# G-U-N/Phased-Consistency-Model

Measured on NVIDIA H100. Metric: distillation steps/sec (SD1.5 PCM-LoRA, bs=8/GPU), higher is better.
Workload: dtype bf16

## Files before the change

pcm_b200/csrc/attn_wg.cu:

```cuda
#include "common.cuh"
#include "wgmma.cuh"
#include "host_common.h"

namespace pcm {

namespace {

constexpr int kAwThreads = 384;
constexpr int kAwStages = 2;
constexpr int kTile = 64 * 128;

struct alignas(64) AttnWgParams {
  CUtensorMap q_map, k_map, v_map;
  bf16* out;
  float* lse;
  int H, Sq, Skv, D;
  long long ldo;
  float c;
};

template <int KB>
__global__ void __launch_bounds__(kAwThreads, 1) attn_fwd_wg_kernel(const __grid_constant__ AttnWgParams p) {
  extern __shared__ uint8_t smem_raw[];
  uint8_t* smem = reinterpret_cast<uint8_t*>((reinterpret_cast<uintptr_t>(smem_raw) + 1023) &
                                             ~static_cast<uintptr_t>(1023));
  uint8_t* sQ = smem;
  uint8_t* sK = sQ + 2 * KB * kTile;
  uint8_t* sV = sK + kAwStages * KB * kTile;
  __shared__ __align__(8) uint64_t q_bar;
  __shared__ __align__(8) uint64_t full_bar[kAwStages];
  __shared__ __align__(8) uint64_t empty_bar[kAwStages];

  const int wg = threadIdx.x >> 7;
  const int b = blockIdx.z, h = blockIdx.y, q0 = blockIdx.x * 128;
  const int nblk = (p.Skv + 63) / 64;
  constexpr uint32_t kv_bytes = 2 * KB * kTile;

  if (threadIdx.x == 0) {
    tma_prefetch_desc(&p.q_map);
    tma_prefetch_desc(&p.k_map);
    tma_prefetch_desc(&p.v_map);
    mbar_init(&q_bar, 1);
    for (int i = 0; i < kAwStages; ++i) {
      mbar_init(&full_bar[i], 1);
      mbar_init(&empty_bar[i], 2);
    }
    fence_barrier_init();
  }
  __syncthreads();
  griddep_sync();

  if (wg == 0) {
    if (threadIdx.x == 0) {
      mbar_arrive_expect_tx(&q_bar, 2 * KB * kTile);
      for (int w = 0; w < 2; ++w)
        for (int kb = 0; kb < KB; ++kb)
          tma_load_3d(sQ + (w * KB + kb) * kTile, &p.q_map, &q_bar, h * p.D + kb * 64, q0 + 64 * w, b);
      for (int j = 0; j < nblk; ++j) {
        const int st = j % kAwStages;
        mbar_wait(&empty_bar[st], ((j / kAwStages) & 1) ^ 1);
        mbar_arrive_expect_tx(&full_bar[st], kv_bytes);
        for (int kb = 0; kb < KB; ++kb) {
          tma_load_3d(sK + (st * KB + kb) * kTile, &p.k_map, &full_bar[st], h * p.D + kb * 64, j * 64, b);
          tma_load_3d(sV + (st * KB + kb) * kTile, &p.v_map, &full_bar[st], h * p.D + kb * 64, j * 64, b);
        }
      }
    }
    return;
  }

  const int cw = wg - 1, et = threadIdx.x & 127, warp = et >> 5, lane = et & 31;
  uint8_t* myQ = sQ + cw * KB * kTile;
  mbar_wait(&q_bar, 0);
  if (p.D < KB * 64) {
    const int c0 = p.D >> 3, nch = KB * 8;
    for (int i = et; i < 64 * nch; i += 128) {
      const int row = i / nch, ch = i - row * nch;
      if (ch < c0) continue;
      const uint32_t a = smem_u32(myQ + (ch >> 3) * kTile) + row * 128 + (((ch & 7) ^ (row & 7)) << 4);
      sts128(a, 0u, 0u, 0u, 0u);
    }
    fence_proxy_async();
  }
  asm volatile("bar.sync %0, 128;" ::"r"(1 + cw) : "memory");

  float o[KB][32];
#pragma unroll
  for (int kb = 0; kb < KB; ++kb)
#pragma unroll
    for (int i = 0; i < 32; ++i) o[kb][i] = 0.f;
  float m_run[2] = {-INFINITY, -INFINITY}, l_run[2] = {0.f, 0.f};
  const uint32_t q_addr = smem_u32(myQ);

  for (int j = 0; j < nblk; ++j) {
    const int st = j % kAwStages;
    mbar_wait(&full_bar[st], (j / kAwStages) & 1);
    const uint32_t k_addr = smem_u32(sK + st * KB * kTile);
    const uint32_t v_addr = smem_u32(sV + st * KB * kTile);
    float s[32];
    wgmma_fence();
#pragma unroll
    for (int kb = 0; kb < KB; ++kb)
#pragma unroll
      for (int k = 0; k < 4; ++k)
        Wgmma<64, 0, 0>::mma(s, wgmma_desc_sw128(q_addr + kb * kTile + k * 32, 16, 1024),
                             wgmma_desc_sw128(k_addr + kb * kTile + k * 32, 16, 1024), (kb | k) != 0 ? 1u : 0u);
    wgmma_commit();
    wgmma_wait<0>();
    wgmma_fence_acc(s);

    const int kbase = j * 64 + 2 * (lane & 3);
    float mx[2] = {-INFINITY, -INFINITY};
#pragma unroll
    for (int i = 0; i < 32; ++i) {
      const int key = kbase + 8 * (i >> 2) + (i & 1);
      const float v = key < p.Skv ? s[i] * p.c : -INFINITY;
      s[i] = v;
      mx[(i >> 1) & 1] = fmaxf(mx[(i >> 1) & 1], v);
    }
    float alpha[2];
#pragma unroll
    for (int r = 0; r < 2; ++r) {
      mx[r] = fmaxf(mx[r], __shfl_xor_sync(0xffffffffu, mx[r], 1));
      mx[r] = fmaxf(mx[r], __shfl_xor_sync(0xffffffffu, mx[r], 2));
      const float mn = fmaxf(m_run[r], mx[r]);
      alpha[r] = exp2f(m_run[r] - mn);
      m_run[r] = mn;
    }
    float rs[2] = {0.f, 0.f};
    uint32_t pa[4][4];
#pragma unroll
    for (int i = 0; i < 32; i += 2) {
      const int r = (i >> 1) & 1;
      const float p0 = exp2f(s[i] - m_run[r]), p1 = exp2f(s[i + 1] - m_run[r]);
      rs[r] += p0 + p1;
      pa[i >> 3][(i & 7) >> 1] = pack_bf16x2(p0, p1);
    }
#pragma unroll
    for (int r = 0; r < 2; ++r) l_run[r] = l_run[r] * alpha[r] + rs[r];
#pragma unroll
    for (int kb = 0; kb < KB; ++kb)
#pragma unroll
      for (int i = 0; i < 32; ++i) o[kb][i] *= alpha[(i >> 1) & 1];

    wgmma_fence();
#pragma unroll
    for (int kk = 0; kk < 4; ++kk)
#pragma unroll
      for (int kb = 0; kb < KB; ++kb)
        wgmma_rs_m64n64<1>(o[kb], pa[kk], wgmma_desc_sw128(v_addr + kb * kTile + kk * 2048, kTile, 1024), 1u);
    wgmma_commit();
    wgmma_wait<0>();
#pragma unroll
    for (int kb = 0; kb < KB; ++kb) wgmma_fence_acc(o[kb]);
    __syncwarp();
    if (et == 0) mbar_arrive(&empty_bar[st]);
  }

#pragma unroll
  for (int r = 0; r < 2; ++r) {
    l_run[r] += __shfl_xor_sync(0xffffffffu, l_run[r], 1);
    l_run[r] += __shfl_xor_sync(0xffffffffu, l_run[r], 2);
  }
  const int row0 = q0 + 64 * cw + 16 * warp + (lane >> 2);
#pragma unroll
  for (int r = 0; r < 2; ++r) {
    const int row = row0 + 8 * r;
    if (row >= p.Sq) continue;
    const float inv = 1.f / l_run[r];
    bf16* orow = p.out + (static_cast<long long>(b) * p.Sq + row) * p.ldo + h * p.D;
#pragma unroll
    for (int kb = 0; kb < KB; ++kb)
#pragma unroll
      for (int q = 0; q < 8; ++q) {
        const int col = kb * 64 + 8 * q + 2 * (lane & 3);
        if (col < p.D)
          *reinterpret_cast<uint32_t*>(orow + col) =
              pack_bf16x2(o[kb][4 * q + 2 * r] * inv, o[kb][4 * q + 2 * r + 1] * inv);
      }
    if ((lane & 3) == 0 && p.lse) p.lse[(static_cast<long long>(b) * p.H + h) * p.Sq + row] = m_run[r] + log2f(l_run[r]);
  }
}

struct alignas(64) AttnBwdParams {
  CUtensorMap fix0_map, fix1_map;
  CUtensorMap str0_map, str1_map;
  const float *lse, *delta;
  bf16 *out0, *out1;
  long long ld0, ld1;
  int H, Sq, Skv, D;
  int n_fix, n_str;
  float c, scale;
};

template <bool KV>
__global__ void __launch_bounds__(kAwThreads, 1) attn_bwd_wg_kernel(const __grid_constant__ AttnBwdParams p) {
  extern __shared__ uint8_t smem_raw[];
  uint8_t* smem = reinterpret_cast<uint8_t*>((reinterpret_cast<uintptr_t>(smem_raw) + 1023) &
                                             ~static_cast<uintptr_t>(1023));
  uint8_t* sF = smem;
  uint8_t* sS = sF + 4 * kTile;
  __shared__ __align__(8) uint64_t f_bar;
// ... 108 lines not shown
#pragma unroll
      for (int e = 0; e < 2; ++e) {
        const int col = 8 * (i >> 2) + 2 * (lane & 3) + e;
        float l, d;
        bool ok;
        if (KV) {
          l = lc[2 * (i >> 2) + e];
          d = dc[2 * (i >> 2) + e];
          ok = rvalid[r];
        } else {
          l = lrow[r];
          d = drow[r];
          ok = j * 64 + col < p.Skv;
        }
        pv[e] = ok ? exp2f(s[i + e] * p.c - l) : 0.f;
        g[e] = pv[e] * (dp[i + e] - d);
      }
      pa[i >> 3][(i & 7) >> 1] = pack_bf16x2(pv[0], pv[1]);
      dsa[i >> 3][(i & 7) >> 1] = pack_bf16x2(g[0], g[1]);
    }
    wgmma_fence();
#pragma unroll
    for (int kk = 0; kk < 4; ++kk) {
      wgmma_rs_m64n64<1>(acc0, dsa[kk], wgmma_desc_sw128(s0 + kk * 2048, kTile, 1024), 1u);
      if (KV) wgmma_rs_m64n64<1>(acc1, pa[kk], wgmma_desc_sw128(s1 + kk * 2048, kTile, 1024), 1u);
    }
    wgmma_commit();
    wgmma_wait<0>();
    wgmma_fence_acc(acc0);
    wgmma_fence_acc(acc1);
    __syncwarp();
    if (et == 0) mbar_arrive(&empty_bar[st]);
  }

#pragma unroll
  for (int r = 0; r < 2; ++r) {
    if (!rvalid[r]) continue;
    const long long row = static_cast<long long>(b) * p.n_fix + frow + 8 * r;
    bf16* o0 = p.out0 + row * p.ld0 + col0;
    bf16* o1 = KV ? p.out1 + row * p.ld1 + col0 : nullptr;
#pragma unroll
    for (int q = 0; q < 8; ++q) {
      const int col = 8 * q + 2 * (lane & 3);
      if (col < p.D) {
        *reinterpret_cast<uint32_t*>(o0 + col) =
            pack_bf16x2(acc0[4 * q + 2 * r] * p.scale, acc0[4 * q + 2 * r + 1] * p.scale);
        if (KV) *reinterpret_cast<uint32_t*>(o1 + col) = pack_bf16x2(acc1[4 * q + 2 * r], acc1[4 * q + 2 * r + 1]);
      }
    }
  }
}

int encode_seq_map(CUtensorMap* m, const void* base, int HD, int S, int B, long long ld) {
  if ((reinterpret_cast<uintptr_t>(base) & 15) != 0 || (ld & 7) != 0)
    return set_error("attention: tensor map base not 16-byte aligned or row stride not a multiple of 8");
  cuuint64_t dims[3] = {static_cast<cuuint64_t>(HD), static_cast<cuuint64_t>(S), static_cast<cuuint64_t>(B)};
  cuuint64_t strides[2] = {static_cast<cuuint64_t>(ld) * 2, static_cast<cuuint64_t>(ld) * 2 * S};
  cuuint32_t box[3] = {64, 64, 1}, estr[3] = {1, 1, 1};
  return encode_tmap(m, base, 3, dims, strides, box, estr);
}

}

int attn_fwd_wg(const void* q, const void* k, const void* v, void* out, float* lse, int B, int H, int Sq,
                int Skv, int D, long long ldq, long long ldk, long long ldv, long long ldo, float scale,
                cudaStream_t stream) {
  if (D % 8 != 0 || D > 128) return 1;
  static AttnWgParams p;
  memset(&p, 0, sizeof(p));
  int rc;
  if ((rc = encode_seq_map(&p.q_map, q, H * D, Sq, B, ldq)) != 0) return rc;
  if ((rc = encode_seq_map(&p.k_map, k, H * D, Skv, B, ldk)) != 0) return rc;
  if ((rc = encode_seq_map(&p.v_map, v, H * D, Skv, B, ldv)) != 0) return rc;
  p.out = reinterpret_cast<bf16*>(out);
  p.lse = lse;
  p.H = H; p.Sq = Sq; p.Skv = Skv; p.D = D; p.ldo = ldo;
  p.c = scale * 1.4426950408889634f;
  const dim3 grid((Sq + 127) / 128, H, B);
  if (D <= 64) {
    const size_t smem = (2 + 2 * kAwStages) * kTile + 1024;
    static bool attr = false;
    if (!attr) {
      CUDA_TRY(cudaFuncSetAttribute(attn_fwd_wg_kernel<1>, cudaFuncAttributeMaxDynamicSharedMemorySize,
                                    static_cast<int>(smem)));
      attr = true;
    }
    CUDA_TRY(launch_pdl(attn_fwd_wg_kernel<1>, grid, dim3(kAwThreads), smem, stream, p));
  } else {
    const size_t smem = 2 * (2 + 2 * kAwStages) * kTile + 1024;
    static bool attr = false;
    if (!attr) {
      CUDA_TRY(cudaFuncSetAttribute(attn_fwd_wg_kernel<2>, cudaFuncAttributeMaxDynamicSharedMemorySize,
                                    static_cast<int>(smem)));
      attr = true;
    }
    CUDA_TRY(launch_pdl(attn_fwd_wg_kernel<2>, grid, dim3(kAwThreads), smem, stream, p));
  }
  CUDA_TRY(cudaGetLastError());
  return 0;
}

int attn_bwd_wg(const void* q, const void* k, const void* v, const void* dout, const float* lse,
                const float* delta, void* dq, void* dk, void* dv, int B, int H, int Sq, int Skv, int D,
                long long ldq, long long ldk, long long ldv, long long ldo, float scale, cudaStream_t stream) {
  if (D % 8 != 0 || D > 64) return 1;
  static AttnBwdParams pk, pq;
  memset(&pk, 0, sizeof(pk));
  int rc;
  if ((rc = encode_seq_map(&pk.fix0_map, k, H * D, Skv, B, ldk)) != 0) return rc;
  if ((rc = encode_seq_map(&pk.fix1_map, v, H * D, Skv, B, ldv)) != 0) return rc;
  if ((rc = encode_seq_map(&pk.str0_map, q, H * D, Sq, B, ldq)) != 0) return rc;
  if ((rc = encode_seq_map(&pk.str1_map, dout, H * D, Sq, B, ldo)) != 0) return rc;
  pk.lse = lse; pk.delta = delta;
  pk.H = H; pk.Sq = Sq; pk.Skv = Skv; pk.D = D;
  pk.c = scale * 1.4426950408889634f;
  pq = pk;
  pk.out0 = reinterpret_cast<bf16*>(dk); pk.ld0 = ldk;
  pk.out1 = reinterpret_cast<bf16*>(dv); pk.ld1 = ldv;
  pk.n_fix = Skv; pk.n_str = Sq; pk.scale = scale;
  pq.fix0_map = pk.str0_map; pq.fix1_map = pk.str1_map;
// ... 21 lines not shown
```

pcm_b200/csrc/common.cuh:

```cuda
#pragma once
#include <cuda.h>
#include <cuda_bf16.h>
#include <cuda_runtime.h>
#include <stdint.h>

namespace pcm {

typedef __nv_bfloat16 bf16;

__device__ __forceinline__ uint32_t smem_u32(const void* p) {
  return static_cast<uint32_t>(__cvta_generic_to_shared(p));
}

__device__ __forceinline__ void sts128(uint32_t addr, uint32_t a, uint32_t b, uint32_t c, uint32_t d) {
  asm volatile("st.shared.v4.b32 [%0], {%1, %2, %3, %4};" ::"r"(addr), "r"(a), "r"(b), "r"(c), "r"(d)
               : "memory");
}
__device__ __forceinline__ float4 lds128(uint32_t addr) {
  float4 v;
  asm volatile("ld.shared.v4.f32 {%0, %1, %2, %3}, [%4];"
               : "=f"(v.x), "=f"(v.y), "=f"(v.z), "=f"(v.w)
               : "r"(addr)
               : "memory");
  return v;
// ... 119 lines not shown
__device__ __forceinline__ void wgmma_fence_acc(float (&d)[R]) {
#pragma unroll
  for (int i = 0; i < R; ++i) asm volatile("" : "+f"(d[i])::"memory");
}

template <int R>
__device__ __forceinline__ void regs_dealloc() {
  asm volatile("setmaxnreg.dec.sync.aligned.u32 %0;" ::"n"(R));
}
template <int R>
__device__ __forceinline__ void regs_alloc() {
  asm volatile("setmaxnreg.inc.sync.aligned.u32 %0;" ::"n"(R));
}

__device__ __forceinline__ uint64_t wgmma_desc_sw128(uint32_t smem_addr, uint32_t lbo_bytes,
                                                     uint32_t sbo_bytes) {
  uint64_t d = 0;
  d |= static_cast<uint64_t>((smem_addr & 0x3FFFF) >> 4);
  d |= static_cast<uint64_t>((lbo_bytes >> 4) & 0x3FFF) << 16;
  d |= static_cast<uint64_t>((sbo_bytes >> 4) & 0x3FFF) << 32;
  d |= static_cast<uint64_t>(1) << 62;
  return d;
}

__device__ __forceinline__ void red_add_v4(float* addr, float a, float b, float c, float d) {
  asm volatile("red.global.add.v4.f32 [%0], {%1, %2, %3, %4};" ::"l"(addr), "f"(a), "f"(b), "f"(c), "f"(d)
               : "memory");
}

__device__ __forceinline__ uint32_t pack_bf16x2(float a, float b) {
  __nv_bfloat162 h = __floats2bfloat162_rn(a, b);
  return *reinterpret_cast<uint32_t*>(&h);
}
__device__ __forceinline__ float2 unpack_bf16x2(uint32_t u) {
  __nv_bfloat162 h = *reinterpret_cast<__nv_bfloat162*>(&u);
  return __bfloat1622float2(h);
}
__device__ __forceinline__ float warp_sum(float v) {
#pragma unroll
  for (int o = 16; o > 0; o >>= 1) v += __shfl_xor_sync(0xffffffffu, v, o);
  return v;
}
__device__ __forceinline__ float warp_max(float v) {
#pragma unroll
  for (int o = 16; o > 0; o >>= 1) v = fmaxf(v, __shfl_xor_sync(0xffffffffu, v, o));
  return v;
}
__device__ __forceinline__ float frcp_approx(float d) {
  float r;
  asm("rcp.approx.ftz.f32 %0, %1;" : "=f"(r) : "f"(d));
  return r;
}
__device__ __forceinline__ float sigmoid_f(float x) { return frcp_approx(1.f + __expf(-x)); }
__device__ __forceinline__ float silu_f(float x) { return x * sigmoid_f(x); }
__device__ __forceinline__ float dsilu_f(float x) {
  const float s = sigmoid_f(x);
  return s * (1.f + x * (1.f - s));
}

}
```

pcm_b200/csrc/host_common.cu:

```cuda
#include "host_common.h"
#include <stdio.h>
#include <stdlib.h>
#include <cudaTypedefs.h>
#include "../../include/pcm_b200.h"

namespace pcm {

static thread_local char g_err[512] = "";

int set_error(const char* msg) {
  snprintf(g_err, sizeof(g_err), "%s", msg);
  return -1;
}
int set_cuda_error(cudaError_t e, const char* what) {
  snprintf(g_err, sizeof(g_err), "CUDA error %d (%s) at %s", static_cast<int>(e),
           cudaGetErrorString(e), what);
  return -2;
}
bool pdl_enabled() {
  static int v = -1;
  if (v < 0) v = getenv("PCM_NO_PDL") ? 0 : 1;
  return v == 1;
}
int num_sms() {
// ... 13 lines not shown
                             CUtensorMapL2promotion, CUtensorMapFloatOOBfill);

static EncodeFn get_encode() {
  static EncodeFn fn = nullptr;
  if (!fn) {
    void* p = nullptr;
    cudaDriverEntryPointQueryResult q;
    if (cudaGetDriverEntryPoint("cuTensorMapEncodeTiled", &p, cudaEnableDefault, &q) ==
            cudaSuccess &&
        q == cudaDriverEntryPointSuccess)
      fn = reinterpret_cast<EncodeFn>(p);
  }
  return fn;
}

int encode_tmap(CUtensorMap* map, const void* base, int rank, const cuuint64_t* dims,
                const cuuint64_t* strides_bytes, const cuuint32_t* box, const cuuint32_t* estr,
                int swizzle_bytes) {
  EncodeFn fn = get_encode();
  if (!fn) return set_error("cuTensorMapEncodeTiled entry point unavailable (no CUDA driver?)");
  CUresult r = fn(map, CU_TENSOR_MAP_DATA_TYPE_BFLOAT16, static_cast<cuuint32_t>(rank),
                  const_cast<void*>(base), dims, strides_bytes, box, estr,
                  CU_TENSOR_MAP_INTERLEAVE_NONE,
                  swizzle_bytes == 64 ? CU_TENSOR_MAP_SWIZZLE_64B : CU_TENSOR_MAP_SWIZZLE_128B,
                  CU_TENSOR_MAP_L2_PROMOTION_L2_256B, CU_TENSOR_MAP_FLOAT_OOB_FILL_NONE);
  if (r != CUDA_SUCCESS) {
    char buf[256];
    snprintf(buf, sizeof(buf),
             "cuTensorMapEncodeTiled failed (%d): rank %d dims [%llu,%llu,%llu,%llu] box "
             "[%u,%u,%u,%u] stride0 %llu",
             static_cast<int>(r), rank, (unsigned long long)dims[0],
             (unsigned long long)(rank > 1 ? dims[1] : 0), (unsigned long long)(rank > 2 ? dims[2] : 0),
             (unsigned long long)(rank > 3 ? dims[3] : 0), box[0], rank > 1 ? box[1] : 0,
             rank > 2 ? box[2] : 0, rank > 3 ? box[3] : 0, (unsigned long long)strides_bytes[0]);
    return set_error(buf);
  }
  return 0;
}

const char* last_error() { return g_err; }

}

extern "C" const char* pcm_last_error(void) { return pcm::last_error(); }
extern "C" int pcm_version(void) { return 1; }
extern "C" int pcm_num_sms(void) { return pcm::num_sms(); }
```

pcm_b200/csrc/wgmma.cuh:

```cuda
#pragma once
#include <stdint.h>

namespace pcm {

template <int N, int TA, int TB>
struct Wgmma;

template <int TA, int TB>
struct Wgmma<32, TA, TB> {
  __device__ __forceinline__ static void mma(float (&d)[16], uint64_t a, uint64_t b, uint32_t acc) {
    asm volatile(
        "{\n\t.reg .pred p;\n\t"
        "setp.ne.b32 p, %18, 0;\n\t"
        "wgmma.mma_async.sync.aligned.m64n32k16.f32.bf16.bf16 "
        "{%0, %1, %2, %3, %4, %5, %6, %7, %8, %9, %10, %11, %12, %13, %14, %15}, "
        "%16, %17, p, 1, 1, %19, %20;\n\t}"
        : "+f"(d[0]), "+f"(d[1]), "+f"(d[2]), "+f"(d[3]), "+f"(d[4]), "+f"(d[5]), "+f"(d[6]), "+f"(d[7]), "+f"(d[8]), "+f"(d[9]), "+f"(d[10]), "+f"(d[11]), "+f"(d[12]), "+f"(d[13]), "+f"(d[14]), "+f"(d[15])
        : "l"(a), "l"(b), "r"(acc), "n"(TA), "n"(TB));
  }
};

template <int TA, int TB>
struct Wgmma<64, TA, TB> {
  __device__ __forceinline__ static void mma(float (&d)[32], uint64_t a, uint64_t b, uint32_t acc) {
// ... 72 lines not shown
        "setp.ne.b32 p, %114, 0;\n\t"
        "wgmma.mma_async.sync.aligned.m64n224k16.f32.bf16.bf16 "
        "{%0, %1, %2, %3, %4, %5, %6, %7, %8, %9, %10, %11, %12, %13, %14, %15, %16, %17, %18, %19, %20, %21, %22, %23, %24, %25, %26, %27, %28, %29, %30, %31, %32, %33, %34, %35, %36, %37, %38, %39, %40, %41, %42, %43, %44, %45, %46, %47, %48, %49, %50, %51, %52, %53, %54, %55, %56, %57, %58, %59, %60, %61, %62, %63, %64, %65, %66, %67, %68, %69, %70, %71, %72, %73, %74, %75, %76, %77, %78, %79, %80, %81, %82, %83, %84, %85, %86, %87, %88, %89, %90, %91, %92, %93, %94, %95, %96, %97, %98, %99, %100, %101, %102, %103, %104, %105, %106, %107, %108, %109, %110, %111}, "
        "%112, %113, p, 1, 1, %115, %116;\n\t}"
        : "+f"(d[0]), "+f"(d[1]), "+f"(d[2]), "+f"(d[3]), "+f"(d[4]), "+f"(d[5]), "+f"(d[6]), "+f"(d[7]), "+f"(d[8]), "+f"(d[9]), "+f"(d[10]), "+f"(d[11]), "+f"(d[12]), "+f"(d[13]), "+f"(d[14]), "+f"(d[15]), "+f"(d[16]), "+f"(d[17]), "+f"(d[18]), "+f"(d[19]), "+f"(d[20]), "+f"(d[21]), "+f"(d[22]), "+f"(d[23]), "+f"(d[24]), "+f"(d[25]), "+f"(d[26]), "+f"(d[27]), "+f"(d[28]), "+f"(d[29]), "+f"(d[30]), "+f"(d[31]), "+f"(d[32]), "+f"(d[33]), "+f"(d[34]), "+f"(d[35]), "+f"(d[36]), "+f"(d[37]), "+f"(d[38]), "+f"(d[39]), "+f"(d[40]), "+f"(d[41]), "+f"(d[42]), "+f"(d[43]), "+f"(d[44]), "+f"(d[45]), "+f"(d[46]), "+f"(d[47]), "+f"(d[48]), "+f"(d[49]), "+f"(d[50]), "+f"(d[51]), "+f"(d[52]), "+f"(d[53]), "+f"(d[54]), "+f"(d[55]), "+f"(d[56]), "+f"(d[57]), "+f"(d[58]), "+f"(d[59]), "+f"(d[60]), "+f"(d[61]), "+f"(d[62]), "+f"(d[63]), "+f"(d[64]), "+f"(d[65]), "+f"(d[66]), "+f"(d[67]), "+f"(d[68]), "+f"(d[69]), "+f"(d[70]), "+f"(d[71]), "+f"(d[72]), "+f"(d[73]), "+f"(d[74]), "+f"(d[75]), "+f"(d[76]), "+f"(d[77]), "+f"(d[78]), "+f"(d[79]), "+f"(d[80]), "+f"(d[81]), "+f"(d[82]), "+f"(d[83]), "+f"(d[84]), "+f"(d[85]), "+f"(d[86]), "+f"(d[87]), "+f"(d[88]), "+f"(d[89]), "+f"(d[90]), "+f"(d[91]), "+f"(d[92]), "+f"(d[93]), "+f"(d[94]), "+f"(d[95]), "+f"(d[96]), "+f"(d[97]), "+f"(d[98]), "+f"(d[99]), "+f"(d[100]), "+f"(d[101]), "+f"(d[102]), "+f"(d[103]), "+f"(d[104]), "+f"(d[105]), "+f"(d[106]), "+f"(d[107]), "+f"(d[108]), "+f"(d[109]), "+f"(d[110]), "+f"(d[111])
        : "l"(a), "l"(b), "r"(acc), "n"(TA), "n"(TB));
  }
};

template <int TA, int TB>
struct Wgmma<256, TA, TB> {
  __device__ __forceinline__ static void mma(float (&d)[128], uint64_t a, uint64_t b, uint32_t acc) {
    asm volatile(
        "{\n\t.reg .pred p;\n\t"
        "setp.ne.b32 p, %130, 0;\n\t"
        "wgmma.mma_async.sync.aligned.m64n256k16.f32.bf16.bf16 "
        "{%0, %1, %2, %3, %4, %5, %6, %7, %8, %9, %10, %11, %12, %13, %14, %15, %16, %17, %18, %19, %20, %21, %22, %23, %24, %25, %26, %27, %28, %29, %30, %31, %32, %33, %34, %35, %36, %37, %38, %39, %40, %41, %42, %43, %44, %45, %46, %47, %48, %49, %50, %51, %52, %53, %54, %55, %56, %57, %58, %59, %60, %61, %62, %63, %64, %65, %66, %67, %68, %69, %70, %71, %72, %73, %74, %75, %76, %77, %78, %79, %80, %81, %82, %83, %84, %85, %86, %87, %88, %89, %90, %91, %92, %93, %94, %95, %96, %97, %98, %99, %100, %101, %102, %103, %104, %105, %106, %107, %108, %109, %110, %111, %112, %113, %114, %115, %116, %117, %118, %119, %120, %121, %122, %123, %124, %125, %126, %127}, "
        "%128, %129, p, 1, 1, %131, %132;\n\t}"
        : "+f"(d[0]), "+f"(d[1]), "+f"(d[2]), "+f"(d[3]), "+f"(d[4]), "+f"(d[5]), "+f"(d[6]), "+f"(d[7]), "+f"(d[8]), "+f"(d[9]), "+f"(d[10]), "+f"(d[11]), "+f"(d[12]), "+f"(d[13]), "+f"(d[14]), "+f"(d[15]), "+f"(d[16]), "+f"(d[17]), "+f"(d[18]), "+f"(d[19]), "+f"(d[20]), "+f"(d[21]), "+f"(d[22]), "+f"(d[23]), "+f"(d[24]), "+f"(d[25]), "+f"(d[26]), "+f"(d[27]), "+f"(d[28]), "+f"(d[29]), "+f"(d[30]), "+f"(d[31]), "+f"(d[32]), "+f"(d[33]), "+f"(d[34]), "+f"(d[35]), "+f"(d[36]), "+f"(d[37]), "+f"(d[38]), "+f"(d[39]), "+f"(d[40]), "+f"(d[41]), "+f"(d[42]), "+f"(d[43]), "+f"(d[44]), "+f"(d[45]), "+f"(d[46]), "+f"(d[47]), "+f"(d[48]), "+f"(d[49]), "+f"(d[50]), "+f"(d[51]), "+f"(d[52]), "+f"(d[53]), "+f"(d[54]), "+f"(d[55]), "+f"(d[56]), "+f"(d[57]), "+f"(d[58]), "+f"(d[59]), "+f"(d[60]), "+f"(d[61]), "+f"(d[62]), "+f"(d[63]), "+f"(d[64]), "+f"(d[65]), "+f"(d[66]), "+f"(d[67]), "+f"(d[68]), "+f"(d[69]), "+f"(d[70]), "+f"(d[71]), "+f"(d[72]), "+f"(d[73]), "+f"(d[74]), "+f"(d[75]), "+f"(d[76]), "+f"(d[77]), "+f"(d[78]), "+f"(d[79]), "+f"(d[80]), "+f"(d[81]), "+f"(d[82]), "+f"(d[83]), "+f"(d[84]), "+f"(d[85]), "+f"(d[86]), "+f"(d[87]), "+f"(d[88]), "+f"(d[89]), "+f"(d[90]), "+f"(d[91]), "+f"(d[92]), "+f"(d[93]), "+f"(d[94]), "+f"(d[95]), "+f"(d[96]), "+f"(d[97]), "+f"(d[98]), "+f"(d[99]), "+f"(d[100]), "+f"(d[101]), "+f"(d[102]), "+f"(d[103]), "+f"(d[104]), "+f"(d[105]), "+f"(d[106]), "+f"(d[107]), "+f"(d[108]), "+f"(d[109]), "+f"(d[110]), "+f"(d[111]), "+f"(d[112]), "+f"(d[113]), "+f"(d[114]), "+f"(d[115]), "+f"(d[116]), "+f"(d[117]), "+f"(d[118]), "+f"(d[119]), "+f"(d[120]), "+f"(d[121]), "+f"(d[122]), "+f"(d[123]), "+f"(d[124]), "+f"(d[125]), "+f"(d[126]), "+f"(d[127])
        : "l"(a), "l"(b), "r"(acc), "n"(TA), "n"(TB));
  }
};

template <int TB>
__device__ __forceinline__ void wgmma_rs_m64n64(float (&d)[32], const uint32_t (&a)[4], uint64_t b, uint32_t acc) {
  asm volatile(
      "{\n\t.reg .pred p;\n\t"
      "setp.ne.b32 p, %37, 0;\n\t"
      "wgmma.mma_async.sync.aligned.m64n64k16.f32.bf16.bf16 "
      "{%0, %1, %2, %3, %4, %5, %6, %7, %8, %9, %10, %11, %12, %13, %14, %15, %16, %17, %18, %19, %20, %21, %22, %23, %24, %25, %26, %27, %28, %29, %30, %31}, "
      "{%32, %33, %34, %35}, %36, p, 1, 1, %38;\n\t}"
      : "+f"(d[0]), "+f"(d[1]), "+f"(d[2]), "+f"(d[3]), "+f"(d[4]), "+f"(d[5]), "+f"(d[6]), "+f"(d[7]), "+f"(d[8]), "+f"(d[9]), "+f"(d[10]), "+f"(d[11]), "+f"(d[12]), "+f"(d[13]), "+f"(d[14]), "+f"(d[15]), "+f"(d[16]), "+f"(d[17]), "+f"(d[18]), "+f"(d[19]), "+f"(d[20]), "+f"(d[21]), "+f"(d[22]), "+f"(d[23]), "+f"(d[24]), "+f"(d[25]), "+f"(d[26]), "+f"(d[27]), "+f"(d[28]), "+f"(d[29]), "+f"(d[30]), "+f"(d[31])
      : "r"(a[0]), "r"(a[1]), "r"(a[2]), "r"(a[3]), "l"(b), "r"(acc), "n"(TB));
}

}
```

Before: 6.343.

## Pipeline QK and PV wgmma in attention forward with head-dim-specialized tiles

Restructures the wgmma attention forward kernel so that the QK^T matmul of block j overlaps the PV matmul of block j-1, and deepens the TMA K/V pipeline to four stages. The kernel is now templated on the padded head dim, using a single wide RS wgmma over V loaded with 32B-swizzled 16-column boxes, and three consumer warpgroups when the head dim is at most 64. It also adds warp-specialized register reallocation, ex2.approx.ftz exponentials, masking only on a ragged final block, and skipping the output rescale when the running max is unchanged. The cost is more shared memory, heavier register pressure, and more complex barrier accounting.

After: 6.617, median of 6. 4.3% higher.

```diff
diff --git a/pcm_b200/csrc/attn_wg.cu b/pcm_b200/csrc/attn_wg.cu
--- a/pcm_b200/csrc/attn_wg.cu
+++ b/pcm_b200/csrc/attn_wg.cu
@@ -8,7 +8,9 @@
 
 constexpr int kAwThreads = 384;
 constexpr int kAwStages = 2;
+constexpr int kFwdStages = 4;
 constexpr int kTile = 64 * 128;
+constexpr int kVBox = 64 * 32;
 
 struct alignas(64) AttnWgParams {
   CUtensorMap q_map, k_map, v_map;
@@ -19,31 +21,43 @@
   float c;
 };
 
-template <int KB>
-__global__ void __launch_bounds__(kAwThreads, 1) attn_fwd_wg_kernel(const __grid_constant__ AttnWgParams p) {
+__host__ __device__ constexpr int fwd_consumers(int DP) { return DP <= 64 ? 3 : 2; }
+
+template <int DP>
+constexpr size_t attn_fwd_smem() {
+  return fwd_consumers(DP) * ((DP + 63) / 64) * kTile + kFwdStages * (((DP + 63) / 64) * kTile + (DP / 16) * kVBox) +
+         1024;
+}
+
+template <int DP>
+__global__ void __launch_bounds__(128 * (fwd_consumers(DP) + 1), 1)
+    attn_fwd_wg_kernel(const __grid_constant__ AttnWgParams p) {
+  constexpr int NC = fwd_consumers(DP);
+  constexpr int KB = (DP + 63) / 64;
+  constexpr int NV = DP / 16;
+  constexpr int kKBytes = KB * kTile, kVBytes = NV * kVBox;
   extern __shared__ uint8_t smem_raw[];
   uint8_t* smem = reinterpret_cast<uint8_t*>((reinterpret_cast<uintptr_t>(smem_raw) + 1023) &
                                              ~static_cast<uintptr_t>(1023));
   uint8_t* sQ = smem;
-  uint8_t* sK = sQ + 2 * KB * kTile;
-  uint8_t* sV = sK + kAwStages * KB * kTile;
+  uint8_t* sK = sQ + NC * kKBytes;
+  uint8_t* sV = sK + kFwdStages * kKBytes;
   __shared__ __align__(8) uint64_t q_bar;
-  __shared__ __align__(8) uint64_t full_bar[kAwStages];
-  __shared__ __align__(8) uint64_t empty_bar[kAwStages];
+  __shared__ __align__(8) uint64_t full_bar[kFwdStages];
+  __shared__ __align__(8) uint64_t empty_bar[kFwdStages];
 
   const int wg = threadIdx.x >> 7;
-  const int b = blockIdx.z, h = blockIdx.y, q0 = blockIdx.x * 128;
+  const int b = blockIdx.z, h = blockIdx.y, q0 = blockIdx.x * 64 * NC;
   const int nblk = (p.Skv + 63) / 64;
-  constexpr uint32_t kv_bytes = 2 * KB * kTile;
 
   if (threadIdx.x == 0) {
     tma_prefetch_desc(&p.q_map);
     tma_prefetch_desc(&p.k_map);
     tma_prefetch_desc(&p.v_map);
     mbar_init(&q_bar, 1);
-    for (int i = 0; i < kAwStages; ++i) {
+    for (int i = 0; i < kFwdStages; ++i) {
       mbar_init(&full_bar[i], 1);
-      mbar_init(&empty_bar[i], 2);
+      mbar_init(&empty_bar[i], NC);
     }
     fence_barrier_init();
   }
@@ -51,26 +65,28 @@
   griddep_sync();
 
   if (wg == 0) {
+    regs_dealloc<NC == 3 ? 32 : 40>();
     if (threadIdx.x == 0) {
-      mbar_arrive_expect_tx(&q_bar, 2 * KB * kTile);
-      for (int w = 0; w < 2; ++w)
+      mbar_arrive_expect_tx(&q_bar, NC * kKBytes);
+      for (int w = 0; w < NC; ++w)
         for (int kb = 0; kb < KB; ++kb)
           tma_load_3d(sQ + (w * KB + kb) * kTile, &p.q_map, &q_bar, h * p.D + kb * 64, q0 + 64 * w, b);
       for (int j = 0; j < nblk; ++j) {
-        const int st = j % kAwStages;
-        mbar_wait(&empty_bar[st], ((j / kAwStages) & 1) ^ 1);
-        mbar_arrive_expect_tx(&full_bar[st], kv_bytes);
-        for (int kb = 0; kb < KB; ++kb) {
-          tma_load_3d(sK + (st * KB + kb) * kTile, &p.k_map, &full_bar[st], h * p.D + kb * 64, j * 64, b);
-          tma_load_3d(sV + (st * KB + kb) * kTile, &p.v_map, &full_bar[st], h * p.D + kb * 64, j * 64, b);
-        }
+        const int st = j % kFwdStages;
+        mbar_wait(&empty_bar[st], ((j / kFwdStages) & 1) ^ 1);
+        mbar_arrive_expect_tx(&full_bar[st], kKBytes + kVBytes);
+        for (int kb = 0; kb < KB; ++kb)
+          tma_load_3d(sK + st * kKBytes + kb * kTile, &p.k_map, &full_bar[st], h * p.D + kb * 64, j * 64, b);
+        for (int n = 0; n < NV; ++n)
+          tma_load_3d(sV + st * kVBytes + n * kVBox, &p.v_map, &full_bar[st], h * p.D + n * 16, j * 64, b);
       }
     }
     return;
   }
 
+  regs_alloc<NC == 3 ? 160 : 232>();
   const int cw = wg - 1, et = threadIdx.x & 127, warp = et >> 5, lane = et & 31;
-  uint8_t* myQ = sQ + cw * KB * kTile;
+  uint8_t* myQ = sQ + cw * kKBytes;
   mbar_wait(&q_bar, 0);
   if (p.D < KB * 64) {
     const int c0 = p.D >> 3, nch = KB * 8;
@@ -84,78 +100,102 @@
   }
   asm volatile("bar.sync %0, 128;" ::"r"(1 + cw) : "memory");
 
-  float o[KB][32];
-#pragma unroll
-  for (int kb = 0; kb < KB; ++kb)
-#pragma unroll
-    for (int i = 0; i < 32; ++i) o[kb][i] = 0.f;
+  float o[DP / 2];
+#pragma unroll
+  for (int i = 0; i < DP / 2; ++i) o[i] = 0.f;
   float m_run[2] = {-INFINITY, -INFINITY}, l_run[2] = {0.f, 0.f};
   const uint32_t q_addr = smem_u32(myQ);
-
-  for (int j = 0; j < nblk; ++j) {
-    const int st = j % kAwStages;
-    mbar_wait(&full_bar[st], (j / kAwStages) & 1);
-    const uint32_t k_addr = smem_u32(sK + st * KB * kTile);
-    const uint32_t v_addr = smem_u32(sV + st * KB * kTile);
-    float s[32];
+  const float c = p.c;
+  const bool ragged = (p.Skv & 63) != 0;
+
+  auto issue_qk = [&](float (&s)[32], int st) {
+    const uint32_t k_addr = smem_u32(sK + st * kKBytes);
     wgmma_fence();
 #pragma unroll
-    for (int kb = 0; kb < KB; ++kb)
-#pragma unroll
-      for (int k = 0; k < 4; ++k)
-        Wgmma<64, 0, 0>::mma(s, wgmma_desc_sw128(q_addr + kb * kTile + k * 32, 16, 1024),
-                             wgmma_desc_sw128(k_addr + kb * kTile + k * 32, 16, 1024), (kb | k) != 0 ? 1u : 0u);
+    for (int k = 0; k < DP / 16; ++k)
+      Wgmma<64, 0, 0>::mma(s, wgmma_desc_sw128(q_addr + (k >> 2) * kTile + (k & 3) * 32, 16, 1024),
+                           wgmma_desc_sw128(k_addr + (k >> 2) * kTile + (k & 3) * 32, 16, 1024), k != 0 ? 1u : 0u);
     wgmma_commit();
-    wgmma_wait<0>();
-    wgmma_fence_acc(s);
-
-    const int kbase = j * 64 + 2 * (lane & 3);
+  };
+  auto issue_pv = [&](const uint32_t (&pa)[4][4], int st) {
+    const uint32_t v_addr = smem_u32(sV + st * kVBytes);
+    wgmma_fence();
+#pragma unroll
+    for (int kk = 0; kk < 4; ++kk) WgmmaRS<DP, 1>::mma(o, pa[kk], wgmma_desc_sw32(v_addr + kk * 512, kVBox, 256), 1u);
+    wgmma_commit();
+  };
+  auto softmax = [&](float (&s)[32], int j, float (&alpha)[2], float (&rs)[2]) {
+#pragma unroll
+    for (int i = 0; i < 32; ++i) s[i] *= c;
+    if (ragged && j == nblk - 1) {
+      const int kbase = j * 64 + 2 * (lane & 3);
+#pragma unroll
+      for (int i = 0; i < 32; ++i)
+        if (kbase + 8 * (i >> 2) + (i & 1) >= p.Skv) s[i] = -INFINITY;
+    }
     float mx[2] = {-INFINITY, -INFINITY};
 #pragma unroll
-    for (int i = 0; i < 32; ++i) {
-      const int key = kbase + 8 * (i >> 2) + (i & 1);
-      const float v = key < p.Skv ? s[i] * p.c : -INFINITY;
-      s[i] = v;
-      mx[(i >> 1) & 1] = fmaxf(mx[(i >> 1) & 1], v);
-    }
-    float alpha[2];
+    for (int i = 0; i < 32; ++i) mx[(i >> 1) & 1] = fmaxf(mx[(i >> 1) & 1], s[i]);
+    float nm[2];
 #pragma unroll
     for (int r = 0; r < 2; ++r) {
       mx[r] = fmaxf(mx[r], __shfl_xor_sync(0xffffffffu, mx[r], 1));
       mx[r] = fmaxf(mx[r], __shfl_xor_sync(0xffffffffu, mx[r], 2));
       const float mn = fmaxf(m_run[r], mx[r]);
-      alpha[r] = exp2f(m_run[r] - mn);
+      alpha[r] = ex2_ftz(m_run[r] - mn);
       m_run[r] = mn;
-    }
-    float rs[2] = {0.f, 0.f};
-    uint32_t pa[4][4];
+      nm[r] = -mn;
+      rs[r] = 0.f;
+    }
 #pragma unroll
     for (int i = 0; i < 32; i += 2) {
       const int r = (i >> 1) & 1;
-      const float p0 = exp2f(s[i] - m_run[r]), p1 = exp2f(s[i + 1] - m_run[r]);
-      rs[r] += p0 + p1;
-      pa[i >> 3][(i & 7) >> 1] = pack_bf16x2(p0, p1);
-    }
+      s[i] = ex2_ftz(s[i] + nm[r]);
+      s[i + 1] = ex2_ftz(s[i + 1] + nm[r]);
+      rs[r] += s[i] + s[i + 1];
+    }
+  };
+  auto pack = [&](uint32_t (&pa)[4][4], const float (&s)[32]) {
+#pragma unroll
+    for (int i = 0; i < 32; i += 2) pa[i >> 3][(i & 7) >> 1] = pack_bf16x2(s[i], s[i + 1]);
+  };
+
+  uint32_t pa[4][4];
+  {
+    mbar_wait(&full_bar[0], 0);
+    float s[32], alpha[2], rs[2];
+    issue_qk(s, 0);
+    wgmma_wait<0>();
+    wgmma_fence_acc(s);
+    softmax(s, 0, alpha, rs);
+    pack(pa, s);
+#pragma unroll
+    for (int r = 0; r < 2; ++r) l_run[r] = rs[r];
+  }
+  for (int j = 1; j < nblk; ++j) {
+    const int st = j % kFwdStages, pst = (j - 1) % kFwdStages;
+    mbar_wait(&full_bar[st], (j / kFwdStages) & 1);
+    float s[32], alpha[2], rs[2];
+    issue_qk(s, st);
+    issue_pv(pa, pst);
+    wgmma_wait<1>();
+    wgmma_fence_acc(s);
+    softmax(s, j, alpha, rs);
+    wgmma_wait<0>();
+    wgmma_fence_acc(o);
+    __syncwarp();
+    if (et == 0) mbar_arrive(&empty_bar[pst]);
 #pragma unroll
     for (int r = 0; r < 2; ++r) l_run[r] = l_run[r] * alpha[r] + rs[r];
-#pragma unroll
-    for (int kb = 0; kb < KB; ++kb)
-#pragma unroll
-      for (int i = 0; i < 32; ++i) o[kb][i] *= alpha[(i >> 1) & 1];
-
-    wgmma_fence();
-#pragma unroll
-    for (int kk = 0; kk < 4; ++kk)
-#pragma unroll
-      for (int kb = 0; kb < KB; ++kb)
-        wgmma_rs_m64n64<1>(o[kb], pa[kk], wgmma_desc_sw128(v_addr + kb * kTile + kk * 2048, kTile, 1024), 1u);
-    wgmma_commit();
-    wgmma_wait<0>();
-#pragma unroll
-    for (int kb = 0; kb < KB; ++kb) wgmma_fence_acc(o[kb]);
-    __syncwarp();
-    if (et == 0) mbar_arrive(&empty_bar[st]);
-  }
+    if (!__all_sync(0xffffffffu, alpha[0] == 1.f && alpha[1] == 1.f)) {
+#pragma unroll
+      for (int i = 0; i < DP / 2; ++i) o[i] *= alpha[(i >> 1) & 1];
+    }
+    pack(pa, s);
+  }
+  issue_pv(pa, (nblk - 1) % kFwdStages);
+  wgmma_wait<0>();
+  wgmma_fence_acc(o);
 
 #pragma unroll
   for (int r = 0; r < 2; ++r) {
@@ -170,14 +210,11 @@
     const float inv = 1.f / l_run[r];
     bf16* orow = p.out + (static_cast<long long>(b) * p.Sq + row) * p.ldo + h * p.D;
 #pragma unroll
-    for (int kb = 0; kb < KB; ++kb)
-#pragma unroll
-      for (int q = 0; q < 8; ++q) {
-        const int col = kb * 64 + 8 * q + 2 * (lane & 3);
-        if (col < p.D)
-          *reinterpret_cast<uint32_t*>(orow + col) =
-              pack_bf16x2(o[kb][4 * q + 2 * r] * inv, o[kb][4 * q + 2 * r + 1] * inv);
-      }
+    for (int q = 0; q < DP / 8; ++q) {
+      const int col = 8 * q + 2 * (lane & 3);
+      if (col < p.D)
+        *reinterpret_cast<uint32_t*>(orow + col) = pack_bf16x2(o[4 * q + 2 * r] * inv, o[4 * q + 2 * r + 1] * inv);
+    }
     if ((lane & 3) == 0 && p.lse) p.lse[(static_cast<long long>(b) * p.H + h) * p.Sq + row] = m_run[r] + log2f(l_run[r]);
   }
 }
@@ -332,8 +369,8 @@
     wgmma_fence();
 #pragma unroll
     for (int kk = 0; kk < 4; ++kk) {
-      wgmma_rs_m64n64<1>(acc0, dsa[kk], wgmma_desc_sw128(s0 + kk * 2048, kTile, 1024), 1u);
-      if (KV) wgmma_rs_m64n64<1>(acc1, pa[kk], wgmma_desc_sw128(s1 + kk * 2048, kTile, 1024), 1u);
+      WgmmaRS<64, 1>::mma(acc0, dsa[kk], wgmma_desc_sw128(s0 + kk * 2048, kTile, 1024), 1u);
+      if (KV) WgmmaRS<64, 1>::mma(acc1, pa[kk], wgmma_desc_sw128(s1 + kk * 2048, kTile, 1024), 1u);
     }
     wgmma_commit();
     wgmma_wait<0>();
@@ -361,15 +398,31 @@
   }
 }
 
-int encode_seq_map(CUtensorMap* m, const void* base, int HD, int S, int B, long long ld) {
+int encode_seq_map(CUtensorMap* m, const void* base, int HD, int S, int B, long long ld, int box_cols = 64,
+                   int swizzle_bytes = 128) {
   if ((reinterpret_cast<uintptr_t>(base) & 15) != 0 || (ld & 7) != 0)
     return set_error("attention: tensor map base not 16-byte aligned or row stride not a multiple of 8");
   cuuint64_t dims[3] = {static_cast<cuuint64_t>(HD), static_cast<cuuint64_t>(S), static_cast<cuuint64_t>(B)};
   cuuint64_t strides[2] = {static_cast<cuuint64_t>(ld) * 2, static_cast<cuuint64_t>(ld) * 2 * S};
-  cuuint32_t box[3] = {64, 64, 1}, estr[3] = {1, 1, 1};
-  return encode_tmap(m, base, 3, dims, strides, box, estr);
-}
-
+  cuuint32_t box[3] = {static_cast<cuuint32_t>(box_cols), 64, 1}, estr[3] = {1, 1, 1};
+  return encode_tmap(m, base, 3, dims, strides, box, estr, swizzle_bytes);
+}
+
+}
+
+template <int DP>
+int launch_attn_fwd_wg(const AttnWgParams& p, int B, cudaStream_t stream) {
+  constexpr int rows = 64 * fwd_consumers(DP);
+  constexpr size_t smem = attn_fwd_smem<DP>();
+  const dim3 grid((p.Sq + rows - 1) / rows, p.H, B);
+  static bool attr = false;
+  if (!attr) {
+    CUDA_TRY(cudaFuncSetAttribute(attn_fwd_wg_kernel<DP>, cudaFuncAttributeMaxDynamicSharedMemorySize,
+                                  static_cast<int>(smem)));
+    attr = true;
+  }
+  CUDA_TRY(launch_pdl(attn_fwd_wg_kernel<DP>, grid, dim3(128 * (fwd_consumers(DP) + 1)), smem, stream, p));
+  return 0;
 }
 
 int attn_fwd_wg(const void* q, const void* k, const void* v, void* out, float* lse, int B, int H, int Sq,
@@ -381,31 +434,22 @@
   int rc;
   if ((rc = encode_seq_map(&p.q_map, q, H * D, Sq, B, ldq)) != 0) return rc;
   if ((rc = encode_seq_map(&p.k_map, k, H * D, Skv, B, ldk)) != 0) return rc;
-  if ((rc = encode_seq_map(&p.v_map, v, H * D, Skv, B, ldv)) != 0) return rc;
+  if ((rc = encode_seq_map(&p.v_map, v, H * D, Skv, B, ldv, 16, 32)) != 0) return rc;
   p.out = reinterpret_cast<bf16*>(out);
   p.lse = lse;
   p.H = H; p.Sq = Sq; p.Skv = Skv; p.D = D; p.ldo = ldo;
   p.c = scale * 1.4426950408889634f;
-  const dim3 grid((Sq + 127) / 128, H, B);
-  if (D <= 64) {
-    const size_t smem = (2 + 2 * kAwStages) * kTile + 1024;
-    static bool attr = false;
-    if (!attr) {
-      CUDA_TRY(cudaFuncSetAttribute(attn_fwd_wg_kernel<1>, cudaFuncAttributeMaxDynamicSharedMemorySize,
-                                    static_cast<int>(smem)));
-      attr = true;
-    }
-    CUDA_TRY(launch_pdl(attn_fwd_wg_kernel<1>, grid, dim3(kAwThreads), smem, stream, p));
-  } else {
-    const size_t smem = 2 * (2 + 2 * kAwStages) * kTile + 1024;
-    static bool attr = false;
-    if (!attr) {
-      CUDA_TRY(cudaFuncSetAttribute(attn_fwd_wg_kernel<2>, cudaFuncAttributeMaxDynamicSharedMemorySize,
-                                    static_cast<int>(smem)));
-      attr = true;
-    }
-    CUDA_TRY(launch_pdl(attn_fwd_wg_kernel<2>, grid, dim3(kAwThreads), smem, stream, p));
-  }
+  switch ((D + 15) / 16 * 16) {
+    case 16: rc = launch_attn_fwd_wg<16>(p, B, stream); break;
+    case 32: rc = launch_attn_fwd_wg<32>(p, B, stream); break;
+    case 48: rc = launch_attn_fwd_wg<48>(p, B, stream); break;
+    case 64: rc = launch_attn_fwd_wg<64>(p, B, stream); break;
+    case 80: rc = launch_attn_fwd_wg<80>(p, B, stream); break;
+    case 96: rc = launch_attn_fwd_wg<96>(p, B, stream); break;
+    case 128: rc = launch_attn_fwd_wg<128>(p, B, stream); break;
+    default: return set_error("attention: no wgmma forward for this head dim");
+  }
+  if (rc) return rc;
   CUDA_TRY(cudaGetLastError());
   return 0;
 }
diff --git a/pcm_b200/csrc/common.cuh b/pcm_b200/csrc/common.cuh
--- a/pcm_b200/csrc/common.cuh
+++ b/pcm_b200/csrc/common.cuh
@@ -165,6 +165,9 @@
   d |= static_cast<uint64_t>(1) << 62;
   return d;
 }
+__device__ __forceinline__ uint64_t wgmma_desc_sw32(uint32_t smem_addr, uint32_t lbo_bytes, uint32_t sbo_bytes) {
+  return wgmma_desc_sw128(smem_addr, lbo_bytes, sbo_bytes) | (static_cast<uint64_t>(3) << 62);
+}
 
 __device__ __forceinline__ void red_add_v4(float* addr, float a, float b, float c, float d) {
   asm volatile("red.global.add.v4.f32 [%0], {%1, %2, %3, %4};" ::"l"(addr), "f"(a), "f"(b), "f"(c), "f"(d)
@@ -192,6 +195,11 @@
 __device__ __forceinline__ float frcp_approx(float d) {
   float r;
   asm("rcp.approx.ftz.f32 %0, %1;" : "=f"(r) : "f"(d));
+  return r;
+}
+__device__ __forceinline__ float ex2_ftz(float x) {
+  float r;
+  asm("ex2.approx.ftz.f32 %0, %1;" : "=f"(r) : "f"(x));
   return r;
 }
 __device__ __forceinline__ float sigmoid_f(float x) { return frcp_approx(1.f + __expf(-x)); }
diff --git a/pcm_b200/csrc/host_common.cu b/pcm_b200/csrc/host_common.cu
--- a/pcm_b200/csrc/host_common.cu
+++ b/pcm_b200/csrc/host_common.cu
@@ -59,7 +59,9 @@
   CUresult r = fn(map, CU_TENSOR_MAP_DATA_TYPE_BFLOAT16, static_cast<cuuint32_t>(rank),
                   const_cast<void*>(base), dims, strides_bytes, box, estr,
                   CU_TENSOR_MAP_INTERLEAVE_NONE,
-                  swizzle_bytes == 64 ? CU_TENSOR_MAP_SWIZZLE_64B : CU_TENSOR_MAP_SWIZZLE_128B,
+                  swizzle_bytes == 32   ? CU_TENSOR_MAP_SWIZZLE_32B
+                  : swizzle_bytes == 64 ? CU_TENSOR_MAP_SWIZZLE_64B
+                                        : CU_TENSOR_MAP_SWIZZLE_128B,
                   CU_TENSOR_MAP_L2_PROMOTION_L2_256B, CU_TENSOR_MAP_FLOAT_OOB_FILL_NONE);
   if (r != CUDA_SUCCESS) {
     char buf[256];
diff --git a/pcm_b200/csrc/wgmma.cuh b/pcm_b200/csrc/wgmma.cuh
--- a/pcm_b200/csrc/wgmma.cuh
+++ b/pcm_b200/csrc/wgmma.cuh
@@ -118,16 +118,105 @@
   }
 };
 
-template <int TB>
-__device__ __forceinline__ void wgmma_rs_m64n64(float (&d)[32], const uint32_t (&a)[4], uint64_t b, uint32_t acc) {
-  asm volatile(
-      "{\n\t.reg .pred p;\n\t"
-      "setp.ne.b32 p, %37, 0;\n\t"
-      "wgmma.mma_async.sync.aligned.m64n64k16.f32.bf16.bf16 "
-      "{%0, %1, %2, %3, %4, %5, %6, %7, %8, %9, %10, %11, %12, %13, %14, %15, %16, %17, %18, %19, %20, %21, %22, %23, %24, %25, %26, %27, %28, %29, %30, %31}, "
-      "{%32, %33, %34, %35}, %36, p, 1, 1, %38;\n\t}"
-      : "+f"(d[0]), "+f"(d[1]), "+f"(d[2]), "+f"(d[3]), "+f"(d[4]), "+f"(d[5]), "+f"(d[6]), "+f"(d[7]), "+f"(d[8]), "+f"(d[9]), "+f"(d[10]), "+f"(d[11]), "+f"(d[12]), "+f"(d[13]), "+f"(d[14]), "+f"(d[15]), "+f"(d[16]), "+f"(d[17]), "+f"(d[18]), "+f"(d[19]), "+f"(d[20]), "+f"(d[21]), "+f"(d[22]), "+f"(d[23]), "+f"(d[24]), "+f"(d[25]), "+f"(d[26]), "+f"(d[27]), "+f"(d[28]), "+f"(d[29]), "+f"(d[30]), "+f"(d[31])
-      : "r"(a[0]), "r"(a[1]), "r"(a[2]), "r"(a[3]), "l"(b), "r"(acc), "n"(TB));
+template <int N, int TB>
+struct WgmmaRS;
+
+template <int TB>
+struct WgmmaRS<16, TB> {
+  __device__ __forceinline__ static void mma(float (&d)[8], const uint32_t (&a)[4], uint64_t b, uint32_t acc) {
+    asm volatile(
+        "{\n\t.reg .pred p;\n\t"
+        "setp.ne.b32 p, %13, 0;\n\t"
+        "wgmma.mma_async.sync.aligned.m64n16k16.f32.bf16.bf16 "
+        "{%0, %1, %2, %3, %4, %5, %6, %7}, "
+        "{%8, %9, %10, %11}, %12, p, 1, 1, %14;\n\t}"
+        : "+f"(d[0]), "+f"(d[1]), "+f"(d[2]), "+f"(d[3]), "+f"(d[4]), "+f"(d[5]), "+f"(d[6]), "+f"(d[7])
+        : "r"(a[0]), "r"(a[1]), "r"(a[2]), "r"(a[3]), "l"(b), "r"(acc), "n"(TB));
+  }
+};
+
+template <int TB>
+struct WgmmaRS<32, TB> {
+  __device__ __forceinline__ static void mma(float (&d)[16], const uint32_t (&a)[4], uint64_t b, uint32_t acc) {
+    asm volatile(
+        "{\n\t.reg .pred p;\n\t"
+        "setp.ne.b32 p, %21, 0;\n\t"
+        "wgmma.mma_async.sync.aligned.m64n32k16.f32.bf16.bf16 "
+        "{%0, %1, %2, %3, %4, %5, %6, %7, %8, %9, %10, %11, %12, %13, %14, %15}, "
+        "{%16, %17, %18, %19}, %20, p, 1, 1, %22;\n\t}"
+        : "+f"(d[0]), "+f"(d[1]), "+f"(d[2]), "+f"(d[3]), "+f"(d[4]), "+f"(d[5]), "+f"(d[6]), "+f"(d[7]), "+f"(d[8]), "+f"(d[9]), "+f"(d[10]), "+f"(d[11]), "+f"(d[12]), "+f"(d[13]), "+f"(d[14]), "+f"(d[15])
+        : "r"(a[0]), "r"(a[1]), "r"(a[2]), "r"(a[3]), "l"(b), "r"(acc), "n"(TB));
+  }
+};
+
+template <int TB>
+struct WgmmaRS<48, TB> {
+  __device__ __forceinline__ static void mma(float (&d)[24], const uint32_t (&a)[4], uint64_t b, uint32_t acc) {
+    asm volatile(
+        "{\n\t.reg .pred p;\n\t"
+        "setp.ne.b32 p, %29, 0;\n\t"
+        "wgmma.mma_async.sync.aligned.m64n48k16.f32.bf16.bf16 "
+        "{%0, %1, %2, %3, %4, %5, %6, %7, %8, %9, %10, %11, %12, %13, %14, %15, %16, %17, %18, %19, %20, %21, %22, %23}, "
+        "{%24, %25, %26, %27}, %28, p, 1, 1, %30;\n\t}"
+        : "+f"(d[0]), "+f"(d[1]), "+f"(d[2]), "+f"(d[3]), "+f"(d[4]), "+f"(d[5]), "+f"(d[6]), "+f"(d[7]), "+f"(d[8]), "+f"(d[9]), "+f"(d[10]), "+f"(d[11]), "+f"(d[12]), "+f"(d[13]), "+f"(d[14]), "+f"(d[15]), "+f"(d[16]), "+f"(d[17]), "+f"(d[18]), "+f"(d[19]), "+f"(d[20]), "+f"(d[21]), "+f"(d[22]), "+f"(d[23])
+        : "r"(a[0]), "r"(a[1]), "r"(a[2]), "r"(a[3]), "l"(b), "r"(acc), "n"(TB));
+  }
+};
+
+template <int TB>
+struct WgmmaRS<64, TB> {
+  __device__ __forceinline__ static void mma(float (&d)[32], const uint32_t (&a)[4], uint64_t b, uint32_t acc) {
+    asm volatile(
+        "{\n\t.reg .pred p;\n\t"
+        "setp.ne.b32 p, %37, 0;\n\t"
+        "wgmma.mma_async.sync.aligned.m64n64k16.f32.bf16.bf16 "
+        "{%0, %1, %2, %3, %4, %5, %6, %7, %8, %9, %10, %11, %12, %13, %14, %15, %16, %17, %18, %19, %20, %21, %22, %23, %24, %25, %26, %27, %28, %29, %30, %31}, "
+        "{%32, %33, %34, %35}, %36, p, 1, 1, %38;\n\t}"
+        : "+f"(d[0]), "+f"(d[1]), "+f"(d[2]), "+f"(d[3]), "+f"(d[4]), "+f"(d[5]), "+f"(d[6]), "+f"(d[7]), "+f"(d[8]), "+f"(d[9]), "+f"(d[10]), "+f"(d[11]), "+f"(d[12]), "+f"(d[13]), "+f"(d[14]), "+f"(d[15]), "+f"(d[16]), "+f"(d[17]), "+f"(d[18]), "+f"(d[19]), "+f"(d[20]), "+f"(d[21]), "+f"(d[22]), "+f"(d[23]), "+f"(d[24]), "+f"(d[25]), "+f"(d[26]), "+f"(d[27]), "+f"(d[28]), "+f"(d[29]), "+f"(d[30]), "+f"(d[31])
+        : "r"(a[0]), "r"(a[1]), "r"(a[2]), "r"(a[3]), "l"(b), "r"(acc), "n"(TB));
+  }
+};
+
+template <int TB>
+struct WgmmaRS<80, TB> {
+  __device__ __forceinline__ static void mma(float (&d)[40], const uint32_t (&a)[4], uint64_t b, uint32_t acc) {
+    asm volatile(
+        "{\n\t.reg .pred p;\n\t"
+        "setp.ne.b32 p, %45, 0;\n\t"
+        "wgmma.mma_async.sync.aligned.m64n80k16.f32.bf16.bf16 "
+        "{%0, %1, %2, %3, %4, %5, %6, %7, %8, %9, %10, %11, %12, %13, %14, %15, %16, %17, %18, %19, %20, %21, %22, %23, %24, %25, %26, %27, %28, %29, %30, %31, %32, %33, %34, %35, %36, %37, %38, %39}, "
+        "{%40, %41, %42, %43}, %44, p, 1, 1, %46;\n\t}"
+        : "+f"(d[0]), "+f"(d[1]), "+f"(d[2]), "+f"(d[3]), "+f"(d[4]), "+f"(d[5]), "+f"(d[6]), "+f"(d[7]), "+f"(d[8]), "+f"(d[9]), "+f"(d[10]), "+f"(d[11]), "+f"(d[12]), "+f"(d[13]), "+f"(d[14]), "+f"(d[15]), "+f"(d[16]), "+f"(d[17]), "+f"(d[18]), "+f"(d[19]), "+f"(d[20]), "+f"(d[21]), "+f"(d[22]), "+f"(d[23]), "+f"(d[24]), "+f"(d[25]), "+f"(d[26]), "+f"(d[27]), "+f"(d[28]), "+f"(d[29]), "+f"(d[30]), "+f"(d[31]), "+f"(d[32]), "+f"(d[33]), "+f"(d[34]), "+f"(d[35]), "+f"(d[36]), "+f"(d[37]), "+f"(d[38]), "+f"(d[39])
+        : "r"(a[0]), "r"(a[1]), "r"(a[2]), "r"(a[3]), "l"(b), "r"(acc), "n"(TB));
+  }
+};
+
+template <int TB>
+struct WgmmaRS<96, TB> {
+  __device__ __forceinline__ static void mma(float (&d)[48], const uint32_t (&a)[4], uint64_t b, uint32_t acc) {
+    asm volatile(
+        "{\n\t.reg .pred p;\n\t"
+        "setp.ne.b32 p, %53, 0;\n\t"
+        "wgmma.mma_async.sync.aligned.m64n96k16.f32.bf16.bf16 "
+        "{%0, %1, %2, %3, %4, %5, %6, %7, %8, %9, %10, %11, %12, %13, %14, %15, %16, %17, %18, %19, %20, %21, %22, %23, %24, %25, %26, %27, %28, %29, %30, %31, %32, %33, %34, %35, %36, %37, %38, %39, %40, %41, %42, %43, %44, %45, %46, %47}, "
+        "{%48, %49, %50, %51}, %52, p, 1, 1, %54;\n\t}"
+        : "+f"(d[0]), "+f"(d[1]), "+f"(d[2]), "+f"(d[3]), "+f"(d[4]), "+f"(d[5]), "+f"(d[6]), "+f"(d[7]), "+f"(d[8]), "+f"(d[9]), "+f"(d[10]), "+f"(d[11]), "+f"(d[12]), "+f"(d[13]), "+f"(d[14]), "+f"(d[15]), "+f"(d[16]), "+f"(d[17]), "+f"(d[18]), "+f"(d[19]), "+f"(d[20]), "+f"(d[21]), "+f"(d[22]), "+f"(d[23]), "+f"(d[24]), "+f"(d[25]), "+f"(d[26]), "+f"(d[27]), "+f"(d[28]), "+f"(d[29]), "+f"(d[30]), "+f"(d[31]), "+f"(d[32]), "+f"(d[33]), "+f"(d[34]), "+f"(d[35]), "+f"(d[36]), "+f"(d[37]), "+f"(d[38]), "+f"(d[39]), "+f"(d[40]), "+f"(d[41]), "+f"(d[42]), "+f"(d[43]), "+f"(d[44]), "+f"(d[45]), "+f"(d[46]), "+f"(d[47])
+        : "r"(a[0]), "r"(a[1]), "r"(a[2]), "r"(a[3]), "l"(b), "r"(acc), "n"(TB));
+  }
+};
+
+template <int TB>
+struct WgmmaRS<128, TB> {
+  __device__ __forceinline__ static void mma(float (&d)[64], const uint32_t (&a)[4], uint64_t b, uint32_t acc) {
+    asm volatile(
+        "{\n\t.reg .pred p;\n\t"
+        "setp.ne.b32 p, %69, 0;\n\t"
+        "wgmma.mma_async.sync.aligned.m64n128k16.f32.bf16.bf16 "
+        "{%0, %1, %2, %3, %4, %5, %6, %7, %8, %9, %10, %11, %12, %13, %14, %15, %16, %17, %18, %19, %20, %21, %22, %23, %24, %25, %26, %27, %28, %29, %30, %31, %32, %33, %34, %35, %36, %37, %38, %39, %40, %41, %42, %43, %44, %45, %46, %47, %48, %49, %50, %51, %52, %53, %54, %55, %56, %57, %58, %59, %60, %61, %62, %63}, "
+        "{%64, %65, %66, %67}, %68, p, 1, 1, %70;\n\t}"
+        : "+f"(d[0]), "+f"(d[1]), "+f"(d[2]), "+f"(d[3]), "+f"(d[4]), "+f"(d[5]), "+f"(d[6]), "+f"(d[7]), "+f"(d[8]), "+f"(d[9]), "+f"(d[10]), "+f"(d[11]), "+f"(d[12]), "+f"(d[13]), "+f"(d[14]), "+f"(d[15]), "+f"(d[16]), "+f"(d[17]), "+f"(d[18]), "+f"(d[19]), "+f"(d[20]), "+f"(d[21]), "+f"(d[22]), "+f"(d[23]), "+f"(d[24]), "+f"(d[25]), "+f"(d[26]), "+f"(d[27]), "+f"(d[28]), "+f"(d[29]), "+f"(d[30]), "+f"(d[31]), "+f"(d[32]), "+f"(d[33]), "+f"(d[34]), "+f"(d[35]), "+f"(d[36]), "+f"(d[37]), "+f"(d[38]), "+f"(d[39]), "+f"(d[40]), "+f"(d[41]), "+f"(d[42]), "+f"(d[43]), "+f"(d[44]), "+f"(d[45]), "+f"(d[46]), "+f"(d[47]), "+f"(d[48]), "+f"(d[49]), "+f"(d[50]), "+f"(d[51]), "+f"(d[52]), "+f"(d[53]), "+f"(d[54]), "+f"(d[55]), "+f"(d[56]), "+f"(d[57]), "+f"(d[58]), "+f"(d[59]), "+f"(d[60]), "+f"(d[61]), "+f"(d[62]), "+f"(d[63])
+        : "r"(a[0]), "r"(a[1]), "r"(a[2]), "r"(a[3]), "l"(b), "r"(acc), "n"(TB));
+  }
+};
+
 }
-
-}
```
